# c-zhou/oatk

Measured on AMD Instinct MI355X. Metric: HiFi Gbases/s through syncasm (syncmer+syncerr) at k=1001 s=31, higher is better.
Workload: dtype u64

## Files before the change

oatk_amd/csrc/api_ec.inc:

```
#include "../../include/oatk_hip_ec.h"
#include "ec.hpp"
#include "ec_wave.hpp"
#include "ec_heavy.hpp"
#include "ec_fused.hpp"
#include "ecgraph.hpp"
#include "ec_seq.hpp"
#include <rocprim/device/device_run_length_encode.hpp>
#include <rocprim/device/device_select.hpp>

struct EcState {
    DevBuf idx_p, idx_n, arc_v, arc_w, arc_ls, arc_cov, arc_del, conv;
    DevBuf scm_del, err_del, vtx_hs_off, vtx_mpos;
    DevBuf copy_n, seg, keep_all, n_blocks, n_blocks64, blk_off, work, out, path_pool, cursor, todo, todo2, slabs, big_slabs, os_slabs;
    DevBuf hyb_slabs[16];
    hipStream_t aux[5] = {nullptr, nullptr, nullptr, nullptr, nullptr};
    hipEvent_t aux_ev[5] = {nullptr, nullptr, nullptr, nullptr, nullptr}, fork_ev = nullptr;
    DevBuf new_n, new_n64, new_off, new_k, new_m, new_s, stats;
    DevBuf live32, live64, live_off, larc, lidx_p, lidx_n;
    DevBuf cov, fwd, key_id, key_sorted, val_occ, occ, occ_off, cov64;
    uint64_t n_vtx = 0, new_tot = 0;
    uint64_t stats_h[12] = {0};
    uint64_t n_work = 0;
    uint32_t staged_over = 0;
    bool done = false;
    DevBuf g_keys, g_keys2, g_ukeys, g_counts, g_nruns, g_nout, g_nout64, g_outoff, g_akey, g_aval, g_skey, g_sval, g_comp, g_flags, g_huge;
    DevBuf g_dist, g_dist2, g_cnt64, g_runoff, g_runls;
    DevBuf g_big, g_keep, g_other, g_lkeys, g_ldist, g_val2, g_wgt2, g_runcov, g_head, g_hpos, g_iota, g_segk, g_segv;
    uint32_t light_c = 0;
    uint64_t g_n_vtx = 0, g_n_arc = 0;
    bool graph_resident = false;
    bool global = false, marked = false;
    uint64_t n_global = 0, imp_used = 0;
    DevBuf g_l2g, g_kid, g_gcov, g_gs;
    bool keep_seq = false;
    bool seq_kept = false, cseq_done = false;
    bool seq_global = false;
// ... 646 lines not shown
    }
    CK(hipStreamSynchronize(ctx->stream));
    CK(hipGetLastError());
    return OATK_OK;
}

extern "C" int oatk_hip_ec_reserve_import(oatk_hip_ctx *ctx, uint64_t bytes)
{
    if (!ctx) return OATK_E_NODEV;
    ctx->import_reserve = bytes < (1u << 20)? (1u << 20) : (bytes + 15) & ~15ULL;
    return OATK_OK;
}

struct EcKnobs {
    int heavy = -1;
    bool stages = false;
    bool serial_tiers = false;
    int32_t step_budget = 1000;
    int32_t min_nw = 0;
    int32_t heavy_cap2 = 0;
    int32_t heavy_fl = 0;
    int32_t waves = 32;
    bool assemble_walk = false;
    bool list_walk = false;
};
static EcKnobs ec_knobs_read()
{
    EcKnobs k;
    auto num = [](const char *n, int32_t lo, int32_t dflt) { const char *e = getenv(n); return e && atoi(e) >= lo? (int32_t) atoi(e) : dflt; };
    { const char *e = getenv("OATK_DEBUG_EC_HEAVY"); k.heavy = e && (e[0] == '0' || e[0] == '1') && !e[1]? e[0] - '0' : -1; }
    k.stages = getenv("OATK_DEBUG_EC_STAGES") != nullptr;
    { const char *e = getenv("OATK_DEBUG_EC_SERIAL_TIERS"); k.serial_tiers = e && e[0] == '1'; }
    k.step_budget = num("OATK_DEBUG_EC_STEP_BUDGET", 1, 1000);
    k.min_nw = num("OATK_DEBUG_EC_FUSED_MIN_NW", 2, 0);
    k.heavy_cap2 = num("OATK_DEBUG_EC_HEAVY_CAP2", 1, 0), k.heavy_fl = num("OATK_DEBUG_EC_HEAVY_FL", 64, 0) & ~7;
    k.waves = num("OATK_DEBUG_EC_WAVES", 1, 32);
    { const char *e = getenv("OATK_DEBUG_EC_ASSEMBLE_WALK"); k.assemble_walk = e && e[0] == '1'; }
    { const char *e = getenv("OATK_DEBUG_EC_LIST_WALK"); k.list_walk = e && e[0] == '1'; }
    return k;
}

namespace oatk {

static const int32_t EC_CAP_T0 = 3072;
static const int32_t EC_CAP_T1 = 16384;
static const int32_t EC_ARC_BUDGET = 512;

struct EcTier { int32_t cap_t, cap_c, cap_w, cap_path, cap_f; uint64_t bytes, slab; bool usable, hybrid; int wpb; };

static int32_t ec_cap_c(int32_t cap_t, int K) { return cap_t + cap_t / 8 + 2 * K + 64; }

static int32_t ec_band_cap(int32_t bwmax, double max_edist)
{
    int64_t ct = max_edist > 0? (int64_t) floor((double) bwmax / max_edist) : 0x3FFFFFFF;
    while (ct > 0 && (int32_t) ceil((double) ct * max_edist) > bwmax) --ct;
    return (int32_t) (ct > 60000? 60000 : ct);
}

static uint64_t ec_wg_per_cu(uint64_t bytes)
{
    const uint64_t n = 160 * 1024 / (bytes + 256);
// ... 75 lines not shown
        CK(hipEventCreateWithFlags(&e->fork_ev, hipEventDisableTiming));
    }
    CK(hipEventRecord(e->fork_ev, ctx->stream));
    return OATK_OK;
}

static int ec_route(oatk_hip_ctx *ctx, EcState *e, uint64_t n_work, const EcRoute &rt, unsigned long long *routed, size_t bytes)
{
    hipLaunchKernelGGL(ec_route_kernel, dim3((unsigned) ((n_work + 256 * ECW_ROUTE_ITEMS - 1) / (256 * ECW_ROUTE_ITEMS))), dim3(256), 0, ctx->stream, e->work.as<EcWork>(), n_work, rt);
    CK(hipMemcpyAsync(routed, rt.cnt[0], bytes, hipMemcpyDeviceToHost, ctx->stream));
    CK(hipStreamSynchronize(ctx->stream));
    return OATK_OK;
}

static int ec_sort_longest_first(oatk_hip_ctx *ctx, EcState *e, uint32_t *list, uint64_t n)
{
    uint32_t *k_in = e->todo2.as<uint32_t>(), *k_out = k_in + (n + 1), *v_out = k_out + (n + 1);
    hipLaunchKernelGGL(ec_route_keys_kernel, dim3((unsigned) ((n + 255) / 256)), dim3(256), 0, ctx->stream, e->work.as<EcWork>(), list, n, k_in);
    size_t tb = 0;
    CK(rocprim::radix_sort_pairs(nullptr, tb, k_in, k_out, list, v_out, n, 0, 32, ctx->stream));
    ENSURE(tmp, tb);
    CK(rocprim::radix_sort_pairs(ctx->tmp.p, tb, k_in, k_out, list, v_out, n, 0, 32, ctx->stream));
    CK(hipMemcpyAsync(list, v_out, n * 4, hipMemcpyDeviceToDevice, ctx->stream));
    return OATK_OK;
}

static int ec_launch_slab_tier(oatk_hip_ctx *ctx, EcState *e, const EcwArgs &base, uint32_t &max_hl, const uint32_t *todo, uint64_t n_todo,
                               unsigned long long *queue, hipStream_t st)
{
    if (max_hl == 0) {
        std::vector<uint32_t> hl(ctx->n_reads);
        CK(hipMemcpy(hl.data(), ctx->hoco_l.p, ctx->n_reads * 4, hipMemcpyDeviceToHost));
        for (uint64_t i = 0; i < ctx->n_reads; ++i) if (hl[i] > max_hl) max_hl = hl[i];
    }
    EcwArgs a = base;
    a.cap_t = (int32_t) max_hl + 64, a.cap_c = ec_cap_c(a.cap_t, ctx->K);
    a.cap_w = 2 * ((int32_t) (max_hl * base.max_edist) + 16) + 16, a.cap_path = ec_cap_c((int32_t) max_hl, ctx->K), a.cap_f = 1 << 22;
    a.todo = todo, a.n_todo = n_todo, a.next = queue, a.skip_l = 0x7FFFFFFF, a.batch = 1;
    a.todo_out = e->todo2.as<uint32_t>(), a.todo_cnt = base.pool_cursor + 63;
    a.slab_bytes = ((uint64_t) ecw_scratch_words(a.cap_t, a.cap_c, a.cap_w, a.cap_path, a.cap_f) * 4 + 63) & ~63ULL;
    uint64_t waves = todo? n_todo : base.n_work;
    if (waves > 1024) waves = 1024;
    if (!waves) return OATK_OK;
    EENSURE(big_slabs, waves * a.slab_bytes);
    a.slabs = e->big_slabs.as<uint8_t>();
    ec_wave_launch<1, 1>(waves, 0, st, a);
// ... 150 lines not shown
    for (int c = 1; c < 4; ++c) if (!H[c].usable) rt.list[c] = list[4], rt.cnt[c] = cur + 4;
    rt.cap[0] = T0.usable? T0.cap_t : -1, rt.cap[1] = H[1].routes? H[1].cap_t : 0, rt.cap[2] = H[2].routes? H[2].cap_t : 0, rt.cap[3] = 0x7FFFFFFF;
    unsigned long long routed[5] = {0, 0, 0, 0, 0}, cnts[5] = {0, 0, 0, 0, 0};
    if (n_work) { int rc = ec_route(ctx, e, n_work, rt, routed, sizeof(routed)); if (rc) return rc; }
    { int rc = ec_fork_side_streams(ctx, e); if (rc) return rc; }
    {
        unsigned long long mx = routed[1] > routed[2]? routed[1] : routed[2];
        mx = routed[3] > mx? routed[3] : mx;
        if (mx <= (4u << 20) && 3 * (mx + 1) > n_work + 1) EENSURE(todo2, 3 * (mx + 1) * 4);
    }
    int used_aux = 0;
    for (int c = 3; c >= 1; --c) {
        if (!routed[c]) continue;
        if (routed[c] > 1 && routed[c] <= (64u << 10)) {
            int rc = ec_sort_longest_first(ctx, e, list[c], routed[c]); if (rc) return rc;
            CK(hipEventRecord(e->fork_ev, ctx->stream));
        }
        hipStream_t st = e->aux[used_aux];
        CK(hipStreamWaitEvent(st, e->fork_ev, 0));
        { int rc = launch_class(c, list[c], routed[c], st); if (rc) return rc; }
        CK(hipEventRecord(e->aux_ev[used_aux], st));
        ++used_aux;
    }
    if (T0.usable && n_work) {
        EcwArgs a = base;
        ec_set_caps(a, T0);
        a.todo = nullptr, a.n_todo = 0, a.next = cur + qslot++, a.skip_l = T0.cap_t, a.batch = ECW_BATCH;
        a.arc_budget = EC_ARC_BUDGET;
        a.todo_out = list[1], a.todo_cnt = cur + 1;
        a.os_words = ec_os_words(T0.cap_c), a.os_slabs = e->os_slabs.as<uint32_t>();
        uint64_t waves = t0_waves;
        const uint64_t groups = (n_work + (uint64_t) a.batch - 1) / (uint64_t) a.batch;
        if (waves > groups) waves = groups;
        ec_launch_lds_tier(T0, waves, ctx->stream, a);
    }
    CK(hipMemcpyAsync(cnts, cur, sizeof(cnts), hipMemcpyDeviceToHost, ctx->stream));
    CK(hipStreamSynchronize(ctx->stream));
    if (cnts[1] > routed[1]) { int rc = launch_class(1, list[1] + routed[1], cnts[1] - routed[1], ctx->stream); if (rc) return rc; }
    n_big = cnts[1] + routed[2] + routed[3] + routed[4];
    for (int i = 0; i < used_aux; ++i) CK(hipStreamWaitEvent(ctx->stream, e->aux_ev[i], 0));
    CK(hipMemcpyAsync(cnts, cur, sizeof(cnts), hipMemcpyDeviceToHost, ctx->stream));
    CK(hipStreamSynchronize(ctx->stream));
    if (kn.stages) fprintf(stderr, "[ec stages] first stage done: %llu blocks go on (classes got %llu + %llu + %llu; %llu past a class that does not fit LDS)\n", cnts[4], cnts[1], routed[2], routed[3], routed[4]);
    if (!cnts[4]) return OATK_OK;
    unsigned long long left = 0;
    { int rc = ec_second_stage(ctx, e, kn, base, list[4], cnts[4], list[1], qslot, hyb_k, left); if (rc) return rc; }
    if (!left) return OATK_OK;
    return ec_launch_slab_tier(ctx, e, base, max_hl, list[1], left, cur + qslot++, ctx->stream);
}

static int ec_solve_tiers(oatk_hip_ctx *ctx, EcState *e, const EcKnobs &kn, const EcwArgs &base, uint32_t &max_hl, uint64_t &n_big)
{
    const int LAST = 3;
    const uint64_t n_work = base.n_work;
    unsigned long long *cur = base.pool_cursor;
    const int32_t t_lo = ctx->ec_cap_t0 > 0? ctx->ec_cap_t0 : EC_CAP_T0, t_hi = ctx->ec_cap_t1 > 0? ctx->ec_cap_t1 : EC_CAP_T1;
    EcTier T[LAST + 1];
    T[0] = ec_lds_tier(t_lo, 32, 2048, false, base.max_edist, ctx->K);
    T[1] = ec_lds_tier(2 * t_lo < t_hi? 2 * t_lo : t_hi, 64, 4096, false, base.max_edist, ctx->K);
    T[2] = ec_lds_tier(t_hi, 0, 0, true, base.max_edist, ctx->K);
    T[LAST] = EcTier{}, T[LAST].usable = true;
    uint64_t os_total = 0, os_next = 0;
    for (int t = 0; t < LAST; ++t) if (T[t].usable) os_total += 3 * (ec_tier_waves(T[t], kn.waves, ctx->n_cu) + ECW_WPB) * ec_os_words(T[t].cap_c);
    EENSURE(os_slabs, os_total * 4 + 64);
    EENSURE(todo, 3 * (n_work + 1) * 4); EENSURE(todo2, (n_work + 1) * 4);
    uint32_t *list[4] = {nullptr, e->todo.as<uint32_t>(), e->todo.as<uint32_t>() + (n_work + 1), e->todo.as<uint32_t>() + 2 * (n_work + 1)};
    int qslot = 4, hyb_k = 0;
    auto next_usable = [&](int t) { int u = t + 1; while (u < LAST && !T[u].usable) ++u; return u; };
    auto launch = [&](int tier, const uint32_t *todo, uint64_t n_todo, hipStream_t st, bool routed, uint64_t max_waves = 0) -> int {
        if (qslot >= 60) { ctx->err = "EC solver: more rounds of left-overs than queue counters (internal)"; return OATK_E_STATE; }
        unsigned long long *queue = cur + qslot++;
        if (kn.stages) fprintf(stderr, "[ec stages] tier %d: %llu blocks%s\n", tier, (unsigned long long) (todo? n_todo : n_work), todo? (routed? " routed by length" : " left over") : "");
        if (tier == LAST) return ec_launch_slab_tier(ctx, e, base, max_hl, todo, n_todo, queue, st);
        const EcTier &t = T[tier];
        EcwArgs a = base;
        ec_set_caps(a, t);
        a.todo = todo, a.n_todo = n_todo, a.next = queue;
        a.skip_l = routed && tier == 0? t.cap_t : 0x7FFFFFFF;
        a.batch = tier == 0? ECW_BATCH : 1;
        const int nx = tier < LAST - 1 && T[LAST - 1].usable? LAST - 1 : next_usable(tier);
        a.todo_out = list[nx], a.todo_cnt = cur + nx;
        uint64_t waves = ec_tier_waves(t, kn.waves, ctx->n_cu);
        a.os_words = ec_os_words(t.cap_c);
        if ((os_next + waves * a.os_words) * 4 > e->os_slabs.cap) { ctx->err = "EC solver: more launches than optimum-consensus slabs (internal)"; return OATK_E_STATE; }
        a.os_slabs = e->os_slabs.as<uint32_t>() + os_next;
        os_next += waves * a.os_words;
        const uint64_t n_items = todo? n_todo : n_work;
        const uint64_t groups = (n_items + (uint64_t) a.batch - 1) / (uint64_t) a.batch;
        if (waves > groups) waves = groups;
        if (max_waves && waves > max_waves) waves = max_waves;
        if (!waves) return OATK_OK;
        if (t.hybrid) {
            void *p = nullptr;
            int rc = ec_slab_buf(ctx, e, hyb_k, (waves + ECW_WPB) * t.slab + 64, st, "the hybrid tier", "slabs", &p); if (rc) return rc;
            a.slabs = (uint8_t *) p, a.slab_bytes = t.slab;
        }
        ec_launch_lds_tier(t, waves, st, a);
        return OATK_OK;
    };
    EcRoute rt;
    for (int t = 0; t <= LAST; ++t) rt.cap[t] = T[t].usable? T[t].cap_t : 0, rt.list[t] = list[t], rt.cnt[t] = cur + t;
    rt.cap[LAST] = 0x7FFFFFFF;
    const bool side_by_side = T[0].usable && !kn.serial_tiers && n_work;
    unsigned long long routed[4] = {0, 0, 0, 0}, done[4] = {0, 0, 0, 0}, cnts[4] = {0, 0, 0, 0};
    int used_aux = 0;
    if (side_by_side) {
        { int rc = ec_route(ctx, e, n_work, rt, routed, sizeof(routed)); if (rc) return rc; }
        { int rc = ec_fork_side_streams(ctx, e); if (rc) return rc; }
        for (int tier = LAST - 1; tier >= 1; --tier) {
            if (!T[tier].usable || !routed[tier]) continue;
            hipStream_t st = e->aux[used_aux];
            CK(hipStreamWaitEvent(st, e->fork_ev, 0));
            { int rc = launch(tier, list[tier], routed[tier], st, true, tier == 1? 2 * (uint64_t) ctx->n_cu : 0); if (rc) return rc; }
            CK(hipEventRecord(e->aux_ev[used_aux], st));
            ++used_aux;
            done[tier] = routed[tier];
        }
    }
    const int first_tier = side_by_side || T[0].usable? 0 : next_usable(0);
    { int rc = launch(first_tier, nullptr, 0, ctx->stream, side_by_side); if (rc) return rc; }
    bool waited_aux = used_aux == 0;
    for (int round = 0; ; ++round) {
        CK(hipMemcpyAsync(cnts, cur, sizeof(cnts), hipMemcpyDeviceToHost, ctx->stream));
        CK(hipStreamSynchronize(ctx->stream));
        if (round == 0) n_big = cnts[1] + cnts[2] + routed[3];
        bool any = false;
        for (int tier = first_tier + 1; tier <= LAST; ++tier) {
            if (!T[tier].usable || cnts[tier] <= done[tier]) continue;
            { int rc = launch(tier, list[tier] + done[tier], cnts[tier] - done[tier], ctx->stream, false); if (rc) return rc; }
            done[tier] = cnts[tier];
            any = true;
        }
        if (!any && waited_aux) break;
        if (!waited_aux) { for (int i = 0; i < used_aux; ++i) CK(hipStreamWaitEvent(ctx->stream, e->aux_ev[i], 0)); waited_aux = true; }
    }
    return OATK_OK;
}

}

extern "C" int oatk_hip_ec_correct(oatk_hip_ctx *ctx, double max_edist)
{
    using namespace oatk;
    if (!ctx) return OATK_E_NODEV;
    if (!ctx->ec || !ctx->ec->marked) { ctx->err = "oatk_hip_ec_correct needs oatk_hip_ec_mark"; return OATK_E_STATE; }
    CK(hipSetDevice(ctx->device));
    EcState *e = ctx->ec;
    e->done = false, e->cseq_done = false;
    const bool keep_seq = e->keep_seq;
    e->seq_kept = false;
    const EcKnobs kn = ec_knobs_read();
    EC_VIEWS();
    EcLive lv;
    bool graph_branches = true;
    {
        uint64_t n_live = 0;
        EENSURE(g_flags, 64);
        CK(hipMemsetAsync(e->g_flags.as<uint32_t>() + 8, 0, 12, ctx->stream));
        EENSURE(live32, (na + 1) * 4); EENSURE(lidx_p, (2 * nv + 1) * 4); EENSURE(lidx_n, (2 * nv + 1) * 4);
        if (na) hipLaunchKernelGGL(ec_live_flag_kernel, blocks(na), dim3(256), 0, ctx->stream, na, (const uint8_t *) e->arc_del.p, e->live32.as<uint32_t>());
        { int rc = ec_exclusive_scan_u32(ctx, e, e->live32, e->live64, e->live_off, na, &n_live); if (rc) return rc; }
        if (n_live >= 0xFFFFFFFFULL) { ctx->err = "error correction: more than 2^32 live arcs"; return OATK_E_ARG; }
        EENSURE(larc, (n_live + 1) * sizeof(EcLiveArc));
        hipLaunchKernelGGL(ec_live_idx_kernel, blocks(2 * nv), dim3(256), 0, ctx->stream, 2 * nv, e->idx_p.as<uint64_t>(), e->idx_n.as<uint32_t>(),
                           e->live_off.as<uint64_t>(), e->lidx_p.as<uint32_t>(), e->lidx_n.as<uint32_t>(), e->g_flags.as<uint32_t>() + 9);
        if (na) hipLaunchKernelGGL(ec_live_arc_kernel, blocks(na), dim3(256), 0, ctx->stream, na, (const uint8_t *) e->arc_del.p, e->live_off.as<uint64_t>(),
                                   e->arc_w.as<uint64_t>(), e->arc_ls.as<uint32_t>(), e->vtx_hs_off.as<uint64_t>(), e->vtx_mpos.as<uint32_t>(),
                                   e->lidx_p.as<uint32_t>(), e->lidx_n.as<uint32_t>(), e->larc.as<EcLiveArc>(), e->g_flags.as<uint32_t>() + 8);
        uint32_t fl[2] = {0, 0};
        CK(hipMemcpyAsync(fl, e->g_flags.as<uint32_t>() + 8, 8, hipMemcpyDeviceToHost, ctx->stream));
        CK(hipStreamSynchronize(ctx->stream));
        const uint32_t no_src = fl[0];
        graph_branches = fl[1] != 0;
        if (no_src && ctx->n_occ) { ctx->err = "error correction: a live vertex has no k-mer on this shard (import it: oatk_hip_ec_import_kmers)"; return OATK_E_STATE; }
        lv.idx_p = e->lidx_p.as<uint32_t>(), lv.idx_n = e->lidx_n.as<uint32_t>(), lv.arc = e->larc.as<EcLiveArc>();
    }

    EENSURE(n_blocks, (nr + 1) * 4);
    const dim3 rblocks((unsigned) ((nr + ECR_READS_PER_BLOCK - 1) / ECR_READS_PER_BLOCK > 0? (nr + ECR_READS_PER_BLOCK - 1) / ECR_READS_PER_BLOCK : 1));
    EENSURE(new_n, (nr + 1) * 4); EENSURE(copy_n, (nr + 1) * 4); EENSURE(keep_all, nr + 1);
    const uint64_t stage_cap = nocc + nr + 1;
    e->staged_over = 0;
    if (kn.list_walk) hipLaunchKernelGGL(ec_count_blocks_wave_kernel, rblocks, dim3(256), 0, ctx->stream, rd, (const uint8_t *) e->scm_del.p, e->n_blocks.as<uint32_t>());
    else {
        static_assert(sizeof(EcSeg) == 8, "a staging entry is one val_occ entry");
        EENSURE(val_occ, stage_cap * sizeof(EcSeg));
// ... 2 lines not shown
        CK(hipMemcpyAsync(&e->staged_over, e->g_flags.as<uint32_t>() + 10, 4, hipMemcpyDeviceToHost, ctx->stream));
    }
    uint64_t n_work = 0;
    { int rc = ec_exclusive_scan_u32(ctx, e, e->n_blocks, e->n_blocks64, e->blk_off, nr, &n_work); if (rc) return rc; }
    if (e->staged_over) { ctx->err = "error correction: a read has more error blocks than syncmers + 1 (the block walk's staging array)"; return OATK_E_STATE; }
    EENSURE(work, (n_work + 1) * sizeof(EcWork)); EENSURE(out, (n_work + 1) * sizeof(EcBlockOut));
    e->n_work = n_work;
    EENSURE(seg, (n_work + 1) * sizeof(EcSeg));
    if (kn.list_walk) hipLaunchKernelGGL(ec_list_blocks_wave_kernel, rblocks, dim3(256), 0, ctx->stream, rd, lv, (const uint8_t *) e->scm_del.p, e->blk_off.as<uint64_t>(), e->work.as<EcWork>(),
                                         e->copy_n.as<uint32_t>(), e->seg.as<EcSeg>(), e->keep_all.as<uint8_t>());
    else hipLaunchKernelGGL(ec_fill_work_kernel, blocks(nr), dim3(256), 0, ctx->stream, rd, lv, e->blk_off.as<uint64_t>(), (const EcSeg *) e->val_occ.as<EcSeg>(), e->work.as<EcWork>(), e->seg.as<EcSeg>());
    if (keep_seq) {
        uint64_t slot_words = 0;
        EENSURE(slot_w, (n_work + 1) * 4); EENSURE(qend, (n_work + 1) * 4);
        if (n_work) hipLaunchKernelGGL(ec_slot_words_kernel, blocks(n_work), dim3(256), 0, ctx->stream, e->work.as<EcWork>(), n_work, max_edist, e->slot_w.as<uint32_t>());
        { int rc = ec_exclusive_scan_u32(ctx, e, e->slot_w, e->slot_w64, e->slot_off, n_work, &slot_words); if (rc) return rc; }
        EENSURE(slots, (slot_words + 4) * 4);
    }
    t_end(ctx, OATK_T_EC_MARK);
    t_begin(ctx, OATK_T_EC_SOLVE);

    const bool heavy = kn.heavy < 0? graph_branches : kn.heavy != 0;
    uint64_t pool_cap = 2 * nocc + (uint64_t) 16384 * ECW_POOL_CHUNK + 4096;
    EENSURE(cursor, 512); EENSURE(stats, 16 * 8);
    uint64_t n_big = 0;
    uint32_t max_hl = 0;
    for (;;) {
        EENSURE(path_pool, pool_cap * 8);
        CK(hipMemsetAsync(e->cursor.p, 0, 512, ctx->stream));
        EcwArgs base = {};
        base.lv = lv, base.rd = rd, base.work = e->work.as<EcWork>(), base.n_work = n_work, base.max_edist = max_edist;
        base.out = e->out.as<EcBlockOut>(), base.path_pool = e->path_pool.as<uint64_t>(), base.pool_cap = pool_cap;
        base.pool_cursor = (unsigned long long *) e->cursor.p;
        if (keep_seq) {
            CK(hipMemsetAsync(e->qend.p, 0, (n_work + 1) * 4, ctx->stream));
            base.seq_qend = e->qend.as<uint32_t>(), base.seq_slots = e->slots.as<uint32_t>(), base.seq_slot_off = e->slot_off.as<uint64_t>();
        }
        if (kn.stages) fprintf(stderr, "[ec stages] the live graph %s: %s\n", graph_branches? "branches" : "does not branch", heavy? "classes with budgets, second stage" : "round 4's tiers");
        { int rc = heavy? ec_solve_classes(ctx, e, kn, base, max_hl, n_big) : ec_solve_tiers(ctx, e, kn, base, max_hl, n_big); if (rc) return rc; }
        unsigned long long fin = 0, used = 0;
        CK(hipMemcpyAsync(&fin, base.pool_cursor + 63, 8, hipMemcpyDeviceToHost, ctx->stream));
        CK(hipStreamSynchronize(ctx->stream));
        if (fin) { ctx->err = "error correction: a block outgrew the large scratch slab (DFS deeper than 4 MiB of frames)"; return OATK_E_NOMEM; }
        CK(hipMemcpyAsync(&used, e->cursor.p, 8, hipMemcpyDeviceToHost, ctx->stream));
        CK(hipStreamSynchronize(ctx->stream));
        if (used <= pool_cap) break;
        pool_cap = used + used / 4 + 4096;
    }

    t_end(ctx, OATK_T_EC_SOLVE);
    t_begin(ctx, OATK_T_EC_REFRESH);
    EENSURE(new_n, (nr + 1) * 4);
    CK(hipMemsetAsync(e->stats.p, 0, 16 * 8, ctx->stream));
    EcAssembleArgs aa;
    aa.rd = rd, aa.scm_del = (const uint8_t *) e->scm_del.p, aa.scm_s = g.scm_s, aa.blk_off = e->blk_off.as<uint64_t>();
// ... 145 lines not shown
```

oatk_amd/csrc/ec_wave.hpp:

```cpp
#pragma once
#include <type_traits>
#include "ec.hpp"

namespace oatk {

__device__ __forceinline__ uint32_t ecw_rev_in_bytes(uint32_t x)
{
    x = ((x >> 2) & 0x33333333u) | ((x & 0x33333333u) << 2);
    return ((x >> 4) & 0x0F0F0F0Fu) | ((x & 0x0F0F0F0Fu) << 4);
}
__device__ __forceinline__ uint32_t ecw_rev16(uint32_t x)
{
    x = __builtin_bitreverse32(x);
    return ((x >> 1) & 0x55555555u) | ((x & 0x55555555u) << 1);
}
__device__ __forceinline__ uint32_t ecw_src16(const uint8_t *hs, uint32_t p)
{
    const uint32_t *w = (const uint32_t *) hs + (p >> 4);
    const uint64_t v = (uint64_t) ecw_rev_in_bytes(w[1]) << 32 | ecw_rev_in_bytes(w[0]);
    return (uint32_t) (v >> ((p & 15u) << 1));
}
__device__ __forceinline__ uint32_t ecw_gather16(const uint8_t *hs, int64_t start, bool desc)
{
    if (!desc) return start >= 0? ecw_src16(hs, (uint32_t) start) : ecw_src16(hs, 0) << ((uint32_t) (-start) << 1);
// ... 267 lines not shown
        v -= (at(4, i >> 6) & bit? 1 : 0) - (at(5, i >> 6) & bit? 1 : 0);
        if (v < best) best = v, bi = i, bj = Q;
    }
    const int32_t band = bw[j];
    if (band >= 0 && best > band) best = band + 1, bi = 0, bj = 0;
    out3[3 * j] = best, out3[3 * j + 1] = bi, out3[3 * j + 2] = bj;
}
#endif


struct EcwArcRegs {
    uint4 a;
    uint2 b;
};
__device__ __forceinline__ EcwArcRegs ecw_arc_load(const EcLiveArc *arc, uint32_t i)
{
    EcwArcRegs r;
    const uint4 *q = (const uint4 *) (arc + i);
    r.a = q[0];
    r.b = *(const uint2 *) (q + 1);
    return r;
}

template <bool KEEP = false>
__device__ bool ecw_solve_block(const EcLive &lv, const EcReads &rd, const EcWork &wk, const EcwScratch &s, double max_edist,
                                uint32_t &status_out, uint32_t &np_out, uint32_t &tried_out, uint32_t &n_path_out, uint32_t &wf_steps_out, uint32_t &wf_diag_out, uint32_t &olen_out)
{
    const int lane = threadIdx.x & 63;
    const int K = rd.K;
    const int32_t tl = wk.l;
    int32_t bw = (int32_t) ceil((double) tl * max_edist);
    if (bw < EC_MIN_ERR_BASE) bw = EC_MIN_ERR_BASE;
    if (ECW_RARE(tl > s.cap_t || 2 * bw + 8 > s.cap_w)) return false;
    EcwArcRegs pre;
    pre.a = make_uint4(0, 0, 0, 0), pre.b = make_uint2(0, 0);
    uint32_t pre_idx = 0xFFFFFFFFu;
    if (wk.ln) pre = ecw_arc_load(lv.arc, wk.lp), pre_idx = wk.lp;
    const uint8_t *hs = rd.hoco_s + ((uint64_t) wk.hs16 << 4);
    auto gather_target = [&](auto nwin, auto rev, int32_t wb) __attribute__((always_inline)) {
        constexpr int NW = decltype(nwin)::value;
        constexpr bool R = decltype(rev)::value;
        uint32_t w0[NW], w1[NW], pp[NW];
#pragma unroll
        for (int u = 0; u < NW; ++u) {
            const int32_t wi = wb + lane + 64 * u;
            const int64_t start = R? (int64_t) wk.beg_pos + tl - 1 - (wi << 4) : (int64_t) wk.beg_pos + (wi << 4);
            pp[u] = ecw_gather16_at(start, R);
            w0[u] = w1[u] = 0;
            if ((wi << 4) < tl) { const uint32_t *q = (const uint32_t *) hs + (pp[u] >> 4); w0[u] = q[0], w1[u] = q[1]; }
        }
#pragma unroll
        for (int u = 0; u < NW; ++u) {
            const int32_t wi = wb + lane + 64 * u;
            const int64_t start = R? (int64_t) wk.beg_pos + tl - 1 - (wi << 4) : (int64_t) wk.beg_pos + (wi << 4);
            if ((wi << 4) < tl) s.ts[wi] = ecw_gather16_fin(w0[u], w1[u], pp[u], start, R);
        }
    };
    auto gather_all = [&](auto rev) __attribute__((always_inline)) {
        if (tl <= 1024) gather_target(std::integral_constant<int, 1>(), rev, 0);
        else if (tl <= 2048) gather_target(std::integral_constant<int, 2>(), rev, 0);
// ... 7 lines not shown
    int32_t score = 0, t_end = 0, q_end = 0;
    EcwWave wv;
    wv.k = s.ka, wv.spare = s.kb, wv.n = 1, wv.d0 = 0;
    if (lane == 0) s.ka[0] = -1, s.c_path[0] = wk.beg_utg;
    int32_t fsz = 0, top = -1, nfr = 0;
    bool vpend = false;
    uint32_t v_arc = 0;
    int32_t v_depth = 0;
    ecw_sync();

    auto push_frame = [&](uint32_t lp, uint32_t ln, int32_t depth) -> bool {
        const int32_t need = ((int32_t) sizeof(EcwFrame) + 4 * wv.n + 7) & ~7;
        if (fsz + need > s.cap_f) return false;
        EcwFrame *f = (EcwFrame *) (s.frames + fsz);
        if (lane == 0) {
            f->arc_i = lp, f->arc_end = lp + ln;
            f->l0 = c_len, f->score = score, f->t_end = t_end, f->q_end = q_end, f->n = wv.n, f->d0 = wv.d0, f->prev_off = top, f->depth = depth;
        }
        int32_t *sv = (int32_t *) (f + 1);
        for (int32_t j = lane; j < wv.n; j += 64) sv[j] = wv.k[j];
        top = fsz;
        fsz += need;
        ++nfr;
        return true;
    };
    if (ECW_LIKELY(wk.ln == 1)) vpend = true, v_arc = wk.lp, v_depth = 0;
    else if (!push_frame(wk.lp, wk.ln, 0)) return false;

    while (nfr > 0 || vpend) {
        ecw_sync();
        uint32_t a;
        int32_t depth;
        if (ECW_LIKELY(vpend)) {
            vpend = false;
            a = v_arc, depth = v_depth;
        } else {
            EcwFrame *f = (EcwFrame *) (s.frames + top);
            a = ecw_uniu(f->arc_i);
            const uint32_t a_end = ecw_uniu(f->arc_end);
            if (ECW_RARE(a == a_end)) {
                fsz = top;
                top = ecw_uni(f->prev_off);
                --nfr;
                continue;
            }
            if (lane == 0) f->arc_i = a + 1;
            depth = ecw_uni(f->depth);
            c_len = ecw_uni(f->l0), score = ecw_uni(f->score), t_end = ecw_uni(f->t_end), q_end = ecw_uni(f->q_end);
            wv.n = ecw_uni(f->n), wv.d0 = ecw_uni(f->d0), wv.k = s.ka, wv.spare = s.kb;
            const int32_t *sv = (const int32_t *) (f + 1);
            for (int32_t j = lane; j < wv.n; j += 64) s.ka[j] = sv[j];
        }
        ++tried;
        if (ECW_RARE(s.arc_budget > 0 && (tried > (uint32_t) s.arc_budget || wf_steps > 2u * (uint32_t) s.arc_budget))) return false;
        if (ECW_RARE(pre_idx != a)) pre = ecw_arc_load(lv.arc, a);
        const uint64_t w = ecw_uniu(pre.a.x);
        const int32_t ls = (int32_t) ecw_uniu(pre.a.y), ext = K - ls;
        const uint32_t w_hs16 = ecw_uniu(pre.a.z), w_mpos = ecw_uniu(pre.a.w), w_lp = ecw_uniu(pre.b.x), w_ln = ecw_uniu(pre.b.y);
        const int32_t t_end0 = t_end;
        if (ECW_RARE(depth + 2 > s.cap_path || c_len + ext > s.cap_c)) return false;
        if (lane == 0) s.c_path[depth + 1] = w;
        int32_t cn = depth + 2;
        pre_idx = 0xFFFFFFFFu;
        if (ECW_LIKELY(w_ln)) pre = ecw_arc_load(lv.arc, w_lp), pre_idx = w_lp;
        {
            const uint8_t *vs = rd.hoco_s + ((uint64_t) w_hs16 << 4);
            const uint32_t pos = w_mpos >> 1;
            const bool asc = (uint32_t) (w & 1ULL) == (w_mpos & 1u);
            const int32_t w0 = c_len >> 4, w1 = (c_len + ext - 1) >> 4;
            for (int32_t wb = w0; wb <= w1; wb += 64) {
                const int32_t wi = wb + lane;
                if (wi > w1) continue;
                const int32_t t0 = (wi << 4) - c_len;
                uint32_t x = asc? ecw_gather16(vs, (int64_t) pos + ls + t0, false) : ecw_gather16(vs, (int64_t) pos + K - 1 - ls - t0, true);
                if (t0 < 0) {
                    const uint32_t keep = (1u << ((uint32_t) (-t0) << 1)) - 1u;
                    x = (s.cs[wi] & keep) | (x & ~keep);
                }
                s.cs[wi] = x;
            }
            c_len += ext;
        }
        ecw_sync();
        if (edist == INT32_MAX && wk.end_utg != EC_NONE && wk.end_utg != w && w_ln == 1 && n_path < EC_MAX_DFS_PATH && c_len - K <= tl + bw && c_len >= bw + 3) {
            vpend = true, v_arc = w_lp, v_depth = depth + 1;
            continue;
        }
        for (;;) {
            ++wf_steps, wf_diag += (uint64_t) wv.n;
            if (ecw_step(s.ts, tl, s.cs, c_len, bw, wv, s.ka, s.kb, t_end, q_end)) break;
            ++score;
            if (ECW_RARE(score > bw)) break;
        }
        t_end += 1, q_end += 1;
        const int32_t ql = c_len;
        const int32_t sc = score + tl - t_end;
        bool new_opt = false;
        if (sc <= bw && (wk.end_utg == EC_NONE || wk.end_utg == w)) {
            status = EC_SUCCESS;
            if (sc <= edist) {
                if (t_end > t_end0) s_edist = edist;
                edist = sc;
                if (wk.end_utg == EC_NONE && q_end < ql) --cn;
                if (ECW_RARE(edist == s_edist)) {
                    bool diff = q_end != o_len;
                    if (!diff) {
                        bool d = false;
                        const int32_t nw = (q_end + 15) >> 4;
                        for (int32_t wi = lane; wi < nw; wi += 64) {
                            uint32_t x = s.cs[wi] ^ s.os[wi];
// ... 51 lines not shown
struct EcwArgs {
    EcLive lv;
    EcReads rd;
    const EcWork *work;
    uint64_t n_work;
    const uint32_t *todo;
    uint64_t n_todo;
    double max_edist;
    uint8_t *slabs;
    uint64_t slab_bytes;
    uint32_t *os_slabs;
    uint64_t os_words;
    int32_t cap_t, cap_c, cap_w, cap_path, cap_f;
    EcBlockOut *out;
    uint64_t *path_pool;
    uint64_t pool_cap;
    unsigned long long *pool_cursor;
    unsigned long long *next;
    uint32_t *todo_out;
    unsigned long long *todo_cnt;
    int32_t skip_l;
    int32_t batch;
    int32_t arc_budget;
    uint32_t *seq_qend;
    uint32_t *seq_slots;
    const uint64_t *seq_slot_off;
};

__host__ __device__ inline uint32_t ec_slot_words(int32_t l, double max_edist)
{
    if (l < EC_MIN_ERR_SEQ_LEN) return 0u;
    int32_t bw = (int32_t) ceil((double) l * max_edist);
    if (bw < EC_MIN_ERR_BASE) bw = EC_MIN_ERR_BASE;
    return (uint32_t) ((l + bw + 15) / 16);
}
__device__ __forceinline__ void ec_keep_seq(const EcwArgs &a, uint64_t wi, uint32_t status, uint32_t o_len, const uint32_t *os, int t, int T)
{
    if (status != EC_SUCCESS && status != EC_AMBISNQ) return;
    const uint64_t s0 = a.seq_slot_off[wi];
    uint32_t nw = (o_len + 15u) >> 4;
    const uint32_t room = (uint32_t) (a.seq_slot_off[wi + 1] - s0);
    if (nw > room) nw = room;
    for (uint32_t j = (uint32_t) t; j < nw; j += (uint32_t) T) a.seq_slots[s0 + j] = os[j];
    if (t == 0) a.seq_qend[wi] = o_len;
}

struct EcRoute {
    int32_t cap[4];
    uint32_t *list[4];
    unsigned long long *cnt[4];
};
#define ECW_ROUTE_ITEMS 8
__global__ void ec_route_keys_kernel(const EcWork *work, const uint32_t *list, uint64_t n, uint32_t *keys)
{
    const uint64_t i = (uint64_t) blockIdx.x * blockDim.x + threadIdx.x;
    if (i < n) keys[i] = ~(uint32_t) work[list[i]].l;
}
__global__ void ec_route_longer_kernel(const EcWork *work, const uint32_t *list, uint64_t n, int32_t cap, unsigned long long *cnt)
{
    const uint64_t i = (uint64_t) blockIdx.x * blockDim.x + threadIdx.x;
    const uint64_t b = __ballot(i < n && work[list[i]].l > cap);
    if ((threadIdx.x & 63) == 0 && b) atomicAdd(cnt, (unsigned long long) __builtin_popcountll(b));
}
__global__ __launch_bounds__(256) void ec_route_kernel(const EcWork *work, uint64_t n_work, EcRoute rt)
{
    __shared__ uint32_t cnt[4], base_lo[4], base_hi[4];
    __shared__ uint32_t stage[4][256 * ECW_ROUTE_ITEMS / 2];
    constexpr uint32_t CAP = 256 * ECW_ROUTE_ITEMS / 2;
    if (threadIdx.x < 4) cnt[threadIdx.x] = 0;
    __syncthreads();
    const uint64_t i0 = (uint64_t) blockIdx.x * (256 * ECW_ROUTE_ITEMS);
#pragma unroll
    for (int k = 0; k < ECW_ROUTE_ITEMS; ++k) {
        const uint64_t i = i0 + (uint64_t) k * 256 + threadIdx.x;
        if (i >= n_work) continue;
        const int32_t l = work[i].l;
        int t = 0;
        while (t < 3 && l > rt.cap[t]) ++t;
        if (t == 0) continue;
// ... 33 lines not shown
    extern __shared__ uint32_t ecw_lds[];
    const int lane = threadIdx.x & 63;
    const uint32_t wave = blockIdx.x * (uint32_t) WPB + ecw_uniu(threadIdx.x >> 6);
    EcwScratch s;
    s.cap_t = a.cap_t, s.cap_c = a.cap_c, s.cap_w = a.cap_w, s.cap_path = a.cap_path, s.cap_f = a.cap_f;
    s.arc_budget = MODE == 0? a.arc_budget : 0;
    uint32_t *const p0 = BIG? (uint32_t *) (a.slabs + (uint64_t) wave * a.slab_bytes)
                            : ecw_lds + (WPB > 1? ecw_uniu(threadIdx.x >> 6) * (MODE == 2? ecw_lds_words_hybrid(a.cap_t, a.cap_c, a.cap_w)
                                                                                                      : ecw_scratch_words(a.cap_t, a.cap_c, a.cap_w, a.cap_path, a.cap_f, false)) : 0u);
    uint32_t *p = p0;
    s.ts = p, p += ecw_words(a.cap_t);
    s.cs = p, p += ecw_words(a.cap_c);
    if (BIG) s.os = p, p += ecw_words(a.cap_c);
    else s.os = a.os_slabs + (uint64_t) wave * a.os_words;
    s.ka = (int32_t *) p, p += a.cap_w + 2;
    s.kb = (int32_t *) p, p += a.cap_w + 2;
    p += (p - p0) & 1;
    if (MODE == 2) p = (uint32_t *) (a.slabs + (uint64_t) wave * a.slab_bytes);
    s.c_path = (uint64_t *) p, p += 2 * a.cap_path;
    s.o_path = (uint64_t *) p, p += 2 * a.cap_path;
    s.frames = (uint8_t *) p;
    const uint64_t total = a.todo? a.n_todo : a.n_work;
    uint64_t pool_at = 0, pool_end = 0;
    for (;;) {
        unsigned long long t0 = 0;
        if (lane == 0) t0 = atomicAdd(a.next, (unsigned long long) a.batch);
        t0 = ecw_uni64(t0);
        if (t0 >= total) break;
        const int cnt = total - t0 < (uint64_t) a.batch? (int) (total - t0) : a.batch;
        uint64_t my_wi = 0;
        uint4 m0 = make_uint4(0, 0, 0, 0), m1 = m0, m2 = m0;
        if (lane < cnt) {
            my_wi = a.todo? a.todo[t0 + lane] : t0 + lane;
            const uint4 *q = (const uint4 *) (a.work + my_wi);
            m0 = q[0], m1 = q[1], m2 = q[2];
        }
        for (int i = 0; i < cnt; ++i) {
            EcWork wk;
            const uint64_t wi = (uint64_t) ecw_lane((uint32_t) (my_wi >> 32), i) << 32 | ecw_lane((uint32_t) my_wi, i);
            wk.beg_utg = (uint64_t) ecw_lane(m0.y, i) << 32 | ecw_lane(m0.x, i);
            wk.end_utg = (uint64_t) ecw_lane(m0.w, i) << 32 | ecw_lane(m0.z, i);
            wk.read = ecw_lane(m1.x, i), wk.beg_pos = ecw_lane(m1.y, i);
            wk.l = (int32_t) ecw_lane(m1.z, i), wk.r = (int32_t) ecw_lane(m1.w, i);
            wk.hs16 = ecw_lane(m2.x, i), wk.lp = ecw_lane(m2.y, i), wk.ln = ecw_lane(m2.z, i), wk.pad = 0;
            if (ECW_RARE(wk.l > a.skip_l)) continue;
            EcBlockOut o;
            o.status = EC_FAILURE, o.np = 0, o.path_off = 0, o.flags = 0, o.short_block = 0, o.tried = 0, o.n_path = 0, o.wf_steps = 0, o.wf_diag = 0, o.tier = (uint32_t) MODE;
            const uint64_t tick0 = MODE != 0? __builtin_amdgcn_s_memrealtime() : 0;
            if (ECW_RARE(wk.l < EC_MIN_ERR_SEQ_LEN)) {
                o.short_block = 1;
            } else {
                uint32_t st = 0, np = 0, o_len = 0;
                if (ECW_RARE(!ecw_solve_block<KEEP>(a.lv, a.rd, wk, s, a.max_edist, st, np, o.tried, o.n_path, o.wf_steps, o.wf_diag, o_len))) {
                    o.flags = 1;
                    if (lane == 0) a.todo_out[atomicAdd(a.todo_cnt, 1ULL)] = (uint32_t) wi;
                } else {
                    o.status = st, o.np = np;
                    if (KEEP) ec_keep_seq(a, wi, st, o_len, s.os, lane, 64);
                    if (st == EC_SUCCESS && np) {
                        if (ECW_RARE(pool_at + np > pool_end)) {
                            const unsigned long long want = np > ECW_POOL_CHUNK? np : ECW_POOL_CHUNK;
                            unsigned long long off = 0;
                            if (lane == 0) off = atomicAdd(a.pool_cursor, want);
                            pool_at = ecw_uni64(off), pool_end = pool_at + want;
                        }
                        o.path_off = pool_at;
                        if (pool_at + np <= a.pool_cap) for (uint32_t j = lane; j < np; j += 64) a.path_pool[pool_at + j] = s.o_path[j];
                        pool_at += np;
                    }
                }
            }
            o.ticks = MODE != 0? (uint32_t) (__builtin_amdgcn_s_memrealtime() - tick0) : 0u;
            if (lane == 0) a.out[wi] = o;
            ecw_sync();
        }
    }
}

}
```

Measured before the change: 378.6.

## Sort EC work queues by source arc and memoize shared path prefixes

```diff
diff --git a/oatk_amd/csrc/api_ec.inc b/oatk_amd/csrc/api_ec.inc
--- a/oatk_amd/csrc/api_ec.inc
+++ b/oatk_amd/csrc/api_ec.inc
@@ -7,11 +7,14 @@
 #include "ec_seq.hpp"
 #include <rocprim/device/device_run_length_encode.hpp>
 #include <rocprim/device/device_select.hpp>
+#include <rocprim/iterator/counting_iterator.hpp>
 
 struct EcState {
     DevBuf idx_p, idx_n, arc_v, arc_w, arc_ls, arc_cov, arc_del, conv;
     DevBuf scm_del, err_del, vtx_hs_off, vtx_mpos;
     DevBuf copy_n, seg, keep_all, n_blocks, n_blocks64, blk_off, work, out, path_pool, cursor, todo, todo2, slabs, big_slabs, os_slabs;
+    DevBuf qkey, qidx, qtmp[4];
+    uint64_t n_live = 0, q_used = 0, qk_used = 0;
     DevBuf hyb_slabs[16];
     hipStream_t aux[5] = {nullptr, nullptr, nullptr, nullptr, nullptr};
     hipEvent_t aux_ev[5] = {nullptr, nullptr, nullptr, nullptr, nullptr}, fork_ev = nullptr;
@@ -704,6 +707,8 @@
     int32_t heavy_fl = 0;
     int32_t waves = 32;
     bool assemble_walk = false;
+    int memo = 2;
+    bool queue_sort = true;
     bool list_walk = false;
 };
 static EcKnobs ec_knobs_read()
@@ -719,6 +724,8 @@
     k.waves = num("OATK_DEBUG_EC_WAVES", 1, 32);
     { const char *e = getenv("OATK_DEBUG_EC_ASSEMBLE_WALK"); k.assemble_walk = e && e[0] == '1'; }
     { const char *e = getenv("OATK_DEBUG_EC_LIST_WALK"); k.list_walk = e && e[0] == '1'; }
+    { const char *e = getenv("OATK_DEBUG_EC_MEMO"); k.memo = e && (e[0] == '0' || e[0] == '1') && !e[1]? e[0] - '0' : 2; }
+    { const char *e = getenv("OATK_DEBUG_EC_QUEUE_SORT"); k.queue_sort = !(e && e[0] == '0' && !e[1]); }
     return k;
 }
 
@@ -840,6 +847,54 @@
     ENSURE(tmp, tb);
     CK(rocprim::radix_sort_pairs(ctx->tmp.p, tb, k_in, k_out, list, v_out, n, 0, 32, ctx->stream));
     CK(hipMemcpyAsync(list, v_out, n * 4, hipMemcpyDeviceToDevice, ctx->stream));
+    return OATK_OK;
+}
+
+static int ec_queue_room(oatk_hip_ctx *ctx, EcState *e, uint64_t n_work)
+{
+    e->q_used = e->qk_used = 0;
+    EENSURE(qkey, (4 * (n_work + 1) + 64) * 4); EENSURE(qidx, 2 * (n_work + 1) * 4);
+    return OATK_OK;
+}
+static int ec_queue_sort(oatk_hip_ctx *ctx, EcState *e, const uint32_t *list, uint64_t n, hipStream_t st, DevBuf &tmp, const uint32_t **sorted)
+{
+    auto bits = [](uint64_t v) { int b = 1; while (b < 64 && (v >> b)) ++b; return b; };
+    const uint64_t end_max = 2 * e->g_n_vtx;
+    const uint32_t lp_max = (uint32_t) e->n_live;
+    const int lb = bits(lp_max), total = lb + 8 >= 32? 32 : (lb + 8 + 7) & ~7;
+    const int eb = bits(end_max) < total - lb? bits(end_max) : total - lb;
+    if (e->q_used + n > e->qidx.cap / 4 || e->qk_used + 2 * (n + 1) > e->qkey.cap / 4) { ctx->err = "EC solver: more sorted queues than room for them (internal)"; return OATK_E_STATE; }
+    uint32_t *v_out = e->qidx.as<uint32_t>() + e->q_used, *k_in = e->qkey.as<uint32_t>() + e->qk_used, *k_out = k_in + (n + 1);
+    e->q_used += n, e->qk_used += 2 * (n + 1);
+    hipLaunchKernelGGL(ec_queue_keys_kernel, dim3((unsigned) ((n + 255) / 256)), dim3(256), 0, st, e->work.as<EcWork>(), list, n, lp_max, end_max, eb, k_in);
+    size_t tb = 0;
+    if (list) {
+        CK(rocprim::radix_sort_pairs(nullptr, tb, k_in, k_out, list, v_out, n, 0, (unsigned) (eb + lb), st));
+        if (!tmp.ensure(tb, st)) { ctx->err = "hipMalloc failed (EC queue sort)"; return OATK_E_NOMEM; }
+        CK(rocprim::radix_sort_pairs(tmp.p, tb, k_in, k_out, list, v_out, n, 0, (unsigned) (eb + lb), st));
+    } else {
+        rocprim::counting_iterator<uint32_t> iota(0);
+        CK(rocprim::radix_sort_pairs(nullptr, tb, k_in, k_out, iota, v_out, n, 0, (unsigned) (eb + lb), st));
+        if (!tmp.ensure(tb, st)) { ctx->err = "hipMalloc failed (EC queue sort)"; return OATK_E_NOMEM; }
+        CK(rocprim::radix_sort_pairs(tmp.p, tb, k_in, k_out, iota, v_out, n, 0, (unsigned) (eb + lb), st));
+    }
+    *sorted = v_out;
+    return OATK_OK;
+}
+static int32_t ec_routed_batch(uint64_t n_todo, uint64_t waves)
+{
+    const uint64_t b = waves? n_todo / (16 * waves) : 1;
+    return (int32_t) (b < 1? 1 : (b > ECW_BATCH? ECW_BATCH : b));
+}
+struct EcMemoLog { int tier; unsigned long long n; int32_t batch; int slot; };
+static int ec_memo_report(oatk_hip_ctx *ctx, EcState *e, const std::vector<EcMemoLog> &log)
+{
+    if (log.empty()) return OATK_OK;
+    unsigned long long c[128];
+    CK(hipMemcpyAsync(c, (unsigned long long *) e->cursor.p + 64, sizeof(c), hipMemcpyDeviceToHost, ctx->stream));
+    CK(hipStreamSynchronize(ctx->stream));
+    for (const EcMemoLog &l : log)
+        fprintf(stderr, "[ec stages] wave solver, tier %d, %llu blocks: batch %d, %llu levels reused, %llu blocks started at their sink\n", l.tier, l.n, (int) l.batch, c[2 * l.slot], c[2 * l.slot + 1]);
     return OATK_OK;
 }
 
@@ -1036,10 +1091,17 @@
         CK(hipEventRecord(e->aux_ev[used_aux], st));
         ++used_aux;
     }
+    std::vector<EcMemoLog> mlog;
     if (T0.usable && n_work) {
         EcwArgs a = base;
         ec_set_caps(a, T0);
         a.todo = nullptr, a.n_todo = 0, a.next = cur + qslot++, a.skip_l = T0.cap_t, a.batch = ECW_BATCH;
+        if (kn.queue_sort && n_work > 1) {
+            { int rc = ec_queue_room(ctx, e, n_work); if (rc) return rc; }
+            { int rc = ec_queue_sort(ctx, e, nullptr, n_work, ctx->stream, ctx->tmp, &a.todo); if (rc) return rc; }
+            a.n_todo = n_work;
+        }
+        if (kn.stages) a.memo_stat = cur + 64 + 2 * mlog.size(), mlog.push_back(EcMemoLog{0, (unsigned long long) n_work, a.batch, (int) mlog.size()});
         a.arc_budget = EC_ARC_BUDGET;
         a.todo_out = list[1], a.todo_cnt = cur + 1;
         a.os_words = ec_os_words(T0.cap_c), a.os_slabs = e->os_slabs.as<uint32_t>();
@@ -1050,6 +1112,7 @@
     }
     CK(hipMemcpyAsync(cnts, cur, sizeof(cnts), hipMemcpyDeviceToHost, ctx->stream));
     CK(hipStreamSynchronize(ctx->stream));
+    if (kn.stages) { int rc = ec_memo_report(ctx, e, mlog); if (rc) return rc; }
     if (cnts[1] > routed[1]) { int rc = launch_class(1, list[1] + routed[1], cnts[1] - routed[1], ctx->stream); if (rc) return rc; }
     n_big = cnts[1] + routed[2] + routed[3] + routed[4];
     for (int i = 0; i < used_aux; ++i) CK(hipStreamWaitEvent(ctx->stream, e->aux_ev[i], 0));
@@ -1080,6 +1143,8 @@
     EENSURE(todo, 3 * (n_work + 1) * 4); EENSURE(todo2, (n_work + 1) * 4);
     uint32_t *list[4] = {nullptr, e->todo.as<uint32_t>(), e->todo.as<uint32_t>() + (n_work + 1), e->todo.as<uint32_t>() + 2 * (n_work + 1)};
     int qslot = 4, hyb_k = 0;
+    std::vector<EcMemoLog> mlog;
+    if (kn.queue_sort) { int rc = ec_queue_room(ctx, e, n_work); if (rc) return rc; }
     auto next_usable = [&](int t) { int u = t + 1; while (u < LAST && !T[u].usable) ++u; return u; };
     auto launch = [&](int tier, const uint32_t *todo, uint64_t n_todo, hipStream_t st, bool routed, uint64_t max_waves = 0) -> int {
         if (qslot >= 60) { ctx->err = "EC solver: more rounds of left-overs than queue counters (internal)"; return OATK_E_STATE; }
@@ -1091,7 +1156,7 @@
         ec_set_caps(a, t);
         a.todo = todo, a.n_todo = n_todo, a.next = queue;
         a.skip_l = routed && tier == 0? t.cap_t : 0x7FFFFFFF;
-        a.batch = tier == 0? ECW_BATCH : 1;
+        a.batch = ECW_BATCH;
         const int nx = tier < LAST - 1 && T[LAST - 1].usable? LAST - 1 : next_usable(tier);
         a.todo_out = list[nx], a.todo_cnt = cur + nx;
         uint64_t waves = ec_tier_waves(t, kn.waves, ctx->n_cu);
@@ -1100,10 +1165,22 @@
         a.os_slabs = e->os_slabs.as<uint32_t>() + os_next;
         os_next += waves * a.os_words;
         const uint64_t n_items = todo? n_todo : n_work;
+        if (tier > 0) {
+            uint64_t w1 = waves < n_items? waves : n_items;
+            if (max_waves && w1 > max_waves) w1 = max_waves;
+            a.batch = ec_routed_batch(n_items, w1);
+        }
+        if (kn.queue_sort && (todo? routed : true) && n_items > 1 && a.batch > 1) {
+            DevBuf *tmp = &ctx->tmp;
+            for (int i = 0; i < 4; ++i) if (st == e->aux[i]) tmp = &e->qtmp[i];
+            { int rc = ec_queue_sort(ctx, e, todo, n_items, st, *tmp, &a.todo); if (rc) return rc; }
+            a.n_todo = n_items;
+        }
         const uint64_t groups = (n_items + (uint64_t) a.batch - 1) / (uint64_t) a.batch;
         if (waves > groups) waves = groups;
         if (max_waves && waves > max_waves) waves = max_waves;
         if (!waves) return OATK_OK;
+        if (kn.stages && mlog.size() < 64) a.memo_stat = cur + 64 + 2 * mlog.size(), mlog.push_back(EcMemoLog{tier, (unsigned long long) n_items, a.batch, (int) mlog.size()});
         if (t.hybrid) {
             void *p = nullptr;
             int rc = ec_slab_buf(ctx, e, hyb_k, (waves + ECW_WPB) * t.slab + 64, st, "the hybrid tier", "slabs", &p); if (rc) return rc;
@@ -1148,6 +1225,7 @@
         if (!any && waited_aux) break;
         if (!waited_aux) { for (int i = 0; i < used_aux; ++i) CK(hipStreamWaitEvent(ctx->stream, e->aux_ev[i], 0)); waited_aux = true; }
     }
+    if (kn.stages) { int rc = ec_memo_report(ctx, e, mlog); if (rc) return rc; }
     return OATK_OK;
 }
 
@@ -1176,6 +1254,7 @@
         { int rc = ec_exclusive_scan_u32(ctx, e, e->live32, e->live64, e->live_off, na, &n_live); if (rc) return rc; }
         if (n_live >= 0xFFFFFFFFULL) { ctx->err = "error correction: more than 2^32 live arcs"; return OATK_E_ARG; }
         EENSURE(larc, (n_live + 1) * sizeof(EcLiveArc));
+        e->n_live = n_live;
         hipLaunchKernelGGL(ec_live_idx_kernel, blocks(2 * nv), dim3(256), 0, ctx->stream, 2 * nv, e->idx_p.as<uint64_t>(), e->idx_n.as<uint32_t>(),
                            e->live_off.as<uint64_t>(), e->lidx_p.as<uint32_t>(), e->lidx_n.as<uint32_t>(), e->g_flags.as<uint32_t>() + 9);
         if (na) hipLaunchKernelGGL(ec_live_arc_kernel, blocks(na), dim3(256), 0, ctx->stream, na, (const uint8_t *) e->arc_del.p, e->live_off.as<uint64_t>(),
@@ -1224,15 +1303,16 @@
 
     const bool heavy = kn.heavy < 0? graph_branches : kn.heavy != 0;
     uint64_t pool_cap = 2 * nocc + (uint64_t) 16384 * ECW_POOL_CHUNK + 4096;
-    EENSURE(cursor, 512); EENSURE(stats, 16 * 8);
+    EENSURE(cursor, 512 + 128 * 8); EENSURE(stats, 16 * 8);
     uint64_t n_big = 0;
     uint32_t max_hl = 0;
     for (;;) {
         EENSURE(path_pool, pool_cap * 8);
-        CK(hipMemsetAsync(e->cursor.p, 0, 512, ctx->stream));
+        CK(hipMemsetAsync(e->cursor.p, 0, 512 + 128 * 8, ctx->stream));
         EcwArgs base = {};
         base.lv = lv, base.rd = rd, base.work = e->work.as<EcWork>(), base.n_work = n_work, base.max_edist = max_edist;
         base.out = e->out.as<EcBlockOut>(), base.path_pool = e->path_pool.as<uint64_t>(), base.pool_cap = pool_cap;
+        base.memo = kn.memo;
         base.pool_cursor = (unsigned long long *) e->cursor.p;
         if (keep_seq) {
             CK(hipMemsetAsync(e->qend.p, 0, (n_work + 1) * 4, ctx->stream));
diff --git a/oatk_amd/csrc/ec_wave.hpp b/oatk_amd/csrc/ec_wave.hpp
--- a/oatk_amd/csrc/ec_wave.hpp
+++ b/oatk_amd/csrc/ec_wave.hpp
@@ -313,8 +313,19 @@
     return r;
 }
 
+struct EcwMemo {
+    uint64_t src, ff_end;
+    int32_t depth;
+    int32_t ff_d;
+    uint32_t ff_arc;
+    int32_t ff_cl0, ff_clp;
+    int32_t mode;
+    uint32_t n_reuse, n_ff;
+    __device__ __forceinline__ void reset() { src = ff_end = EC_NONE, depth = 0, ff_d = 0, ff_arc = 0, ff_cl0 = ff_clp = 0; }
+};
+
 template <bool KEEP = false>
-__device__ bool ecw_solve_block(const EcLive &lv, const EcReads &rd, const EcWork &wk, const EcwScratch &s, double max_edist,
+__device__ bool ecw_solve_block(const EcLive &lv, const EcReads &rd, const EcWork &wk, const EcwScratch &s, double max_edist, EcwMemo &mm,
                                 uint32_t &status_out, uint32_t &np_out, uint32_t &tried_out, uint32_t &n_path_out, uint32_t &wf_steps_out, uint32_t &wf_diag_out, uint32_t &olen_out)
 {
     const int lane = threadIdx.x & 63;
@@ -323,10 +334,21 @@
     int32_t bw = (int32_t) ceil((double) tl * max_edist);
     if (bw < EC_MIN_ERR_BASE) bw = EC_MIN_ERR_BASE;
     if (ECW_RARE(tl > s.cap_t || 2 * bw + 8 > s.cap_w)) return false;
+    bool m_live = false;
+    if (mm.mode) {
+        if (ECW_LIKELY(wk.ln == 1)) {
+            if (wk.beg_utg != mm.src) mm.reset(), mm.src = wk.beg_utg;
+            m_live = true;
+        } else mm.reset();
+    }
+    const bool ff = mm.mode > 1 && m_live && mm.ff_d > 0 && wk.end_utg == mm.ff_end && mm.depth >= mm.ff_d && mm.ff_cl0 >= bw + 3 && mm.ff_clp - K <= tl + bw;
+    bool ff_walk = mm.mode > 1 && m_live && wk.end_utg != EC_NONE;
+    int32_t cl0 = ff? mm.ff_cl0 : 0;
+    const uint32_t arc0 = ff? mm.ff_arc : wk.lp;
     EcwArcRegs pre;
     pre.a = make_uint4(0, 0, 0, 0), pre.b = make_uint2(0, 0);
     uint32_t pre_idx = 0xFFFFFFFFu;
-    if (wk.ln) pre = ecw_arc_load(lv.arc, wk.lp), pre_idx = wk.lp;
+    if (wk.ln) pre = ecw_arc_load(lv.arc, arc0), pre_idx = arc0;
     const uint8_t *hs = rd.hoco_s + ((uint64_t) wk.hs16 << 4);
     auto gather_target = [&](auto nwin, auto rev, int32_t wb) __attribute__((always_inline)) {
         constexpr int NW = decltype(nwin)::value;
@@ -380,10 +402,15 @@
         top = fsz;
         fsz += need;
         ++nfr;
+        m_live = false;
         return true;
     };
-    if (ECW_LIKELY(wk.ln == 1)) vpend = true, v_arc = wk.lp, v_depth = 0;
+    if (ECW_LIKELY(wk.ln == 1)) vpend = true, v_arc = arc0, v_depth = 0;
     else if (!push_frame(wk.lp, wk.ln, 0)) return false;
+    if (ff) {
+        v_depth = mm.ff_d, tried = (uint32_t) mm.ff_d, c_len = mm.ff_clp;
+        ++mm.n_ff;
+    }
 
     while (nfr > 0 || vpend) {
         ecw_sync();
@@ -421,7 +448,10 @@
         int32_t cn = depth + 2;
         pre_idx = 0xFFFFFFFFu;
         if (ECW_LIKELY(w_ln)) pre = ecw_arc_load(lv.arc, w_lp), pre_idx = w_lp;
-        {
+        if (ECW_LIKELY(m_live && depth < mm.depth)) {
+            c_len += ext;
+            ++mm.n_reuse;
+        } else {
             const uint8_t *vs = rd.hoco_s + ((uint64_t) w_hs16 << 4);
             const uint32_t pos = w_mpos >> 1;
             const bool asc = (uint32_t) (w & 1ULL) == (w_mpos & 1u);
@@ -438,12 +468,16 @@
                 s.cs[wi] = x;
             }
             c_len += ext;
-        }
-        ecw_sync();
+            if (m_live && depth == mm.depth) ++mm.depth;
+            ecw_sync();
+        }
+        if (depth == 0) cl0 = c_len;
+        if (ff_walk && w == wk.end_utg && depth > 0) mm.ff_end = wk.end_utg, mm.ff_d = depth, mm.ff_arc = a, mm.ff_cl0 = cl0, mm.ff_clp = c_len - ext;
         if (edist == INT32_MAX && wk.end_utg != EC_NONE && wk.end_utg != w && w_ln == 1 && n_path < EC_MAX_DFS_PATH && c_len - K <= tl + bw && c_len >= bw + 3) {
             vpend = true, v_arc = w_lp, v_depth = depth + 1;
             continue;
         }
+        ff_walk = false;
         for (;;) {
             ++wf_steps, wf_diag += (uint64_t) wv.n;
             if (ecw_step(s.ts, tl, s.cs, c_len, bw, wv, s.ka, s.kb, t_end, q_end)) break;
@@ -541,6 +575,8 @@
     int32_t skip_l;
     int32_t batch;
     int32_t arc_budget;
+    int32_t memo;
+    unsigned long long *memo_stat;
     uint32_t *seq_qend;
     uint32_t *seq_slots;
     const uint64_t *seq_slot_off;
@@ -574,6 +610,15 @@
 {
     const uint64_t i = (uint64_t) blockIdx.x * blockDim.x + threadIdx.x;
     if (i < n) keys[i] = ~(uint32_t) work[list[i]].l;
+}
+__global__ void ec_queue_keys_kernel(const EcWork *work, const uint32_t *list, uint64_t n, uint32_t lp_max, uint64_t end_max, int eb, uint32_t *keys)
+{
+    const uint64_t i = (uint64_t) blockIdx.x * blockDim.x + threadIdx.x;
+    if (i >= n) return;
+    const EcWork *w = work + (list? list[i] : i);
+    const uint32_t lp = w->lp < lp_max? w->lp : lp_max;
+    const uint64_t en = w->end_utg < end_max? w->end_utg : end_max;
+    keys[i] = (uint32_t) ((uint64_t) lp << eb | (en & ((1ULL << eb) - 1ULL)));
 }
 __global__ void ec_route_longer_kernel(const EcWork *work, const uint32_t *list, uint64_t n, int32_t cap, unsigned long long *cnt)
 {
@@ -653,11 +698,14 @@
     s.frames = (uint8_t *) p;
     const uint64_t total = a.todo? a.n_todo : a.n_work;
     uint64_t pool_at = 0, pool_end = 0;
+    EcwMemo mm;
+    mm.mode = a.memo, mm.n_reuse = mm.n_ff = 0;
     for (;;) {
         unsigned long long t0 = 0;
         if (lane == 0) t0 = atomicAdd(a.next, (unsigned long long) a.batch);
         t0 = ecw_uni64(t0);
         if (t0 >= total) break;
+        mm.reset();
         const int cnt = total - t0 < (uint64_t) a.batch? (int) (total - t0) : a.batch;
         uint64_t my_wi = 0;
         uint4 m0 = make_uint4(0, 0, 0, 0), m1 = m0, m2 = m0;
@@ -682,7 +730,7 @@
                 o.short_block = 1;
             } else {
                 uint32_t st = 0, np = 0, o_len = 0;
-                if (ECW_RARE(!ecw_solve_block<KEEP>(a.lv, a.rd, wk, s, a.max_edist, st, np, o.tried, o.n_path, o.wf_steps, o.wf_diag, o_len))) {
+                if (ECW_RARE(!ecw_solve_block<KEEP>(a.lv, a.rd, wk, s, a.max_edist, mm, st, np, o.tried, o.n_path, o.wf_steps, o.wf_diag, o_len))) {
                     o.flags = 1;
                     if (lane == 0) a.todo_out[atomicAdd(a.todo_cnt, 1ULL)] = (uint32_t) wi;
                 } else {
@@ -706,6 +754,10 @@
             ecw_sync();
         }
     }
-}
-
-}
+    if (a.memo_stat && lane == 0 && (mm.n_reuse | mm.n_ff)) {
+        atomicAdd(a.memo_stat, (unsigned long long) mm.n_reuse);
+        atomicAdd(a.memo_stat + 1, (unsigned long long) mm.n_ff);
+    }
+}
+
+}
```

New measurement: 389.7 (median of 6 runs). 1.03x the previous value.
